# cuulee/reporter

Hardware: AMD Instinct MI355X
Metric: GPS probes matched/sec (whole node) (higher is better)
Workload: dtype f64; 1 GPU; c2; graph=metro, nodes=1048576, directed_edges=3527937, osmlr_segments=1361487, traces_per_gpu=10000, streams=1, device_batches=1, output_segments=1688548

## Files before the change

### reporter_amd/csrc/otr_kernels.h

```cpp
#pragma once
#include <cstddef>
#include <type_traits>

#include "otr_device.h"
#include "otr_mincode.h"
#include "otr_pred.h"
#include "otr_report.h"

#ifndef OTR_CAP1
#define OTR_CAP1 160
#endif
#ifndef OTR_LOAD1
#define OTR_LOAD1 7
#endif
#ifndef OTR_E1CAP
#define OTR_E1CAP 360
#endif
#ifndef OTR_E1LOAD
#define OTR_E1LOAD 14
#endif

namespace otr {

struct BatchDev {
  int32_t n_traces;
  const int64_t* trace_off;
  const double* lat;
  const double* lon;
  const int64_t* time;
  const float* acc;
  const uint8_t* mode;
};

__global__ void k_select_states(BatchDev b, ModeParams mp, int64_t* state_cnt, const int64_t* state_off,
                                int64_t* state_probe, int32_t* state_trace) {
  int t = blockIdx.x * blockDim.x + threadIdx.x;
  if (t >= b.n_traces) return;
  const int64_t lo = b.trace_off[t], hi = b.trace_off[t + 1];
  const MatchParams& P = mp.m[b.mode[t] < OTR_MODES ? b.mode[t] : 0];
  int64_t cnt = 0;
  int64_t base = state_off ? state_off[t] : 0;
  double la_last = 0.0, lo_last = 0.0;
  double la_n = lo < hi ? b.lat[lo] : 0.0, lo_n = lo < hi ? b.lon[lo] : 0.0;
  for (int64_t i = lo; i < hi; ++i) {
    const double la = la_n, lg = lo_n;
    if (i + 1 < hi) {
      la_n = b.lat[i + 1];
      lo_n = b.lon[i + 1];
    }
    const bool st = (i == lo || i == hi - 1) || gc_dist(la_last, lo_last, la, lg) >= P.interpolation_distance;
    if (st) {
      if (state_off) {
        state_probe[base + cnt] = i;
        state_trace[base + cnt] = t;
      }
      ++cnt;
      la_last = la;
      lo_last = lg;
    }
  }
  if (!state_off) state_cnt[t] = cnt;
}

struct CandBuf {
  uint32_t* edge;
  double* p;
  double* sqd;
  int32_t* count;
  double* radius;
};

__device__ inline bool cand_less(double da, uint32_t ea, double db, uint32_t eb) {
  return da < db || (da == db && ea < eb);
}

__device__ inline bool project_edge(const DevGraph& g, uint4 rec, uint4 pts01, uint4 pts23, uint32_t mode_bit,
                                    double plat, double plon, double mpl, double r2, int64_t* sr_out, int64_t* sc_out,
                                    double* d2_out, double* frac_out, unsigned long long* tests) {
  if (!(rec.w & mode_bit)) return false;
  double best = __builtin_huge_val();
  double best_along = 0.0, bqx = 0.0, bqy = 0.0, acc = 0.0;
  const uint32_t k0 = rec.y, k1 = rec.z;
  constexpr uint32_t kPre = 4;
  const int2 pre0 = make_int2((int)pts01.x, (int)pts01.y);
  int2 q1 = make_int2((int)pts01.z, (int)pts01.w);
  int2 q2 = make_int2((int)pts23.x, (int)pts23.y);
  int2 q3 = make_int2((int)pts23.z, (int)pts23.w);
  int2 pa = pre0;
  for (uint32_t k = k0; k + 1 < k1; ++k) {
    const uint32_t i = k + 1 - k0;
    int2 pb;
    if (i < kPre) {
      pb = q1;
      q1 = q2;
      q2 = q3;
    } else {
      pb = g.shape_ll[k + 1];
    }
    const double ax = (e6(pa.y) - plon) * mpl;
    const double ay = (e6(pa.x) - plat) * kMetersPerDeg;
    const double bx = (e6(pb.y) - plon) * mpl;
    const double by = (e6(pb.x) - plat) * kMetersPerDeg;
    const double dx = bx - ax, dy = by - ay;
    const double l2 = dx * dx + dy * dy;
    double t = 0.0;
    if (l2 > 0.0) {
      t = -(ax * dx + ay * dy) / l2;
      if (t < 0.0) t = 0.0;
      if (t > 1.0) t = 1.0;
    }
    const double qx = ax + t * dx, qy = ay + t * dy;
    const double d2 = qx * qx + qy * qy;
    const double sl = sqrt(l2);
    if (d2 < best) {
      best = d2;
      best_along = acc + t * sl;
      bqx = qx;
      bqy = qy;
    }
    acc = acc + sl;
    pa = pb;
  }
  *tests += k1 - k0 - 1;
  if (!(best <= r2)) return false;
  const double slat = plat + bqy / kMetersPerDeg, slon = plon + bqx / mpl;
  *sr_out = (int64_t)floor((slat - g.grid_min_lat) / g.grid_cell_deg);
  *sc_out = (int64_t)floor((slon - g.grid_min_lon) / g.grid_cell_deg);
  *d2_out = best;
  *frac_out = acc > 0.0 ? best_along / acc : 0.0;
  return true;
}

__device__ inline uint32_t wave_sum_u32(uint32_t v) {
  v += (uint32_t)__builtin_amdgcn_update_dpp(0, (int)v, 0x111, 0xf, 0xf, false);
  v += (uint32_t)__builtin_amdgcn_update_dpp(0, (int)v, 0x112, 0xf, 0xf, false);
  v += (uint32_t)__builtin_amdgcn_update_dpp(0, (int)v, 0x114, 0xf, 0xf, false);
  v += (uint32_t)__builtin_amdgcn_update_dpp(0, (int)v, 0x118, 0xf, 0xf, false);
  v += (uint32_t)__builtin_amdgcn_update_dpp(0, (int)v, 0x142, 0xa, 0xf, false);
  v += (uint32_t)__builtin_amdgcn_update_dpp(0, (int)v, 0x143, 0xc, 0xf, false);
  return (uint32_t)__builtin_amdgcn_readlane((int)v, 63);
}

__device__ inline uint32_t wave_min_u32(uint32_t v) {
  const int I = -1;
  auto mn = [](uint32_t a, int b) { return a < (uint32_t)b ? a : (uint32_t)b; };
  v = mn(v, __builtin_amdgcn_update_dpp(I, (int)v, 0x111, 0xf, 0xf, false));
  v = mn(v, __builtin_amdgcn_update_dpp(I, (int)v, 0x112, 0xf, 0xf, false));
  v = mn(v, __builtin_amdgcn_update_dpp(I, (int)v, 0x114, 0xf, 0xf, false));
  v = mn(v, __builtin_amdgcn_update_dpp(I, (int)v, 0x118, 0xf, 0xf, false));
  v = mn(v, __builtin_amdgcn_update_dpp(I, (int)v, 0x142, 0xa, 0xf, false));
  v = mn(v, __builtin_amdgcn_update_dpp(I, (int)v, 0x143, 0xc, 0xf, false));
  return (uint32_t)__builtin_amdgcn_readlane((int)v, 63);
}

__host__ __device__ constexpr bool old_rounds(int g) { return g == 8; }

template <int G>
struct Grp {
  static constexpr int GL = OTR_WAVE / G;
  __device__ static int g() { return G == 1 ? 0 : (int)threadIdx.x / GL; }
  __device__ static int gl() { return G == 1 ? (int)threadIdx.x : (int)threadIdx.x % GL; }
  __device__ static unsigned long long mine(unsigned long long m) {
    return G == 1 ? m : (m >> (GL * g())) & ((1ull << GL) - 1ull);
  }
  __device__ static int prefix(unsigned long long m) {
    if (G == 1) return prefix_count(m);
    return __popcll(mine(m) & ((1ull << gl()) - 1ull));
  }
  __device__ static int count(unsigned long long m) { return __popcll(mine(m)); }
  __device__ static int umax(int v) {
    if (G == 1) return __builtin_amdgcn_readfirstlane(v);
    if (G == 8) {
      int m = __builtin_amdgcn_readlane(v, 0);
#pragma unroll
      for (int q = 1; q < 8; ++q) {
        const int x = __builtin_amdgcn_readlane(v, q * GL);
        m = x > m ? x : m;
      }
      return m;
    }
    const int a = __builtin_amdgcn_readlane(v, 0), b = __builtin_amdgcn_readlane(v, GL);
    if (G == 2) return a > b ? a : b;
    const int c = __builtin_amdgcn_readlane(v, 2 * GL), d = __builtin_amdgcn_readlane(v, 3 * GL);
    const int ab = a > b ? a : b, cd = c > d ? c : d;
    return ab > cd ? ab : cd;
  }
  __device__ static bool all(bool v) {
    if (G == 8) {
      bool r = true;
#pragma unroll
      for (int q = 0; q < 8; ++q) r = r && __builtin_amdgcn_readlane((int)v, q * GL) != 0;
      return r;
    }
    return __ballot(!v) == 0ull;
  }
  __device__ static uint32_t min_u32(uint32_t v) {
    if (G == 1) return wave_min_u32(v);
    if (G == 8) {
#pragma unroll
      for (int o = 1; o < 8; o <<= 1) {
        const uint32_t x = (uint32_t)__shfl_xor((int)v, o, 8);
        v = x < v ? x : v;
      }
      return v;
    }
    const int I = -1;
    auto mn = [](uint32_t a, int b) { return a < (uint32_t)b ? a : (uint32_t)b; };
    v = mn(v, __builtin_amdgcn_update_dpp(I, (int)v, 0x111, 0xf, 0xf, false));
    v = mn(v, __builtin_amdgcn_update_dpp(I, (int)v, 0x112, 0xf, 0xf, false));
    v = mn(v, __builtin_amdgcn_update_dpp(I, (int)v, 0x114, 0xf, 0xf, false));
    v = mn(v, __builtin_amdgcn_update_dpp(I, (int)v, 0x118, 0xf, 0xf, false));
    if (G == 4) {
      const uint32_t a = (uint32_t)__builtin_amdgcn_readlane((int)v, 15);
      const uint32_t b = (uint32_t)__builtin_amdgcn_readlane((int)v, 31);
      const uint32_t c = (uint32_t)__builtin_amdgcn_readlane((int)v, 47);
      const uint32_t d = (uint32_t)__builtin_amdgcn_readlane((int)v, 63);
      const int q = g();
      return q == 0 ? a : (q == 1 ? b : (q == 2 ? c : d));
    }
    v = mn(v, __builtin_amdgcn_update_dpp(I, (int)v, 0x142, 0xa, 0xf, false));
    const uint32_t a = (uint32_t)__builtin_amdgcn_readlane((int)v, 31);
    const uint32_t b = (uint32_t)__builtin_amdgcn_readlane((int)v, 63);
    return g() ? b : a;
  }
};

constexpr int kWin = 16;
#ifndef OTR_CAND2_WAVES
#define OTR_CAND2_WAVES 5
#endif

template <int G>
__global__ __launch_bounds__(64) __attribute__((amdgpu_waves_per_eu(G == 2 ? OTR_CAND2_WAVES : 8, 8))) void k_candidates(
    DevGraph g, BatchDev b, ModeParams mp, int64_t n_states, const int64_t* state_probe, const int32_t* state_trace,
    CandBuf out, unsigned long long* counters) {
  using Gr = Grp<G>;
  constexpr int GL = Gr::GL;
  constexpr int LB = 2 * GL;
  __shared__ double s_d2[G][LB];
  __shared__ double s_p[G][LB];
  __shared__ uint32_t s_e[G][LB];
  __shared__ uint32_t s_bnd[G][kWin][kWin + 1];
  __shared__ uint32_t s_pre[G][kWin + 1];
  const int gi = Gr::g(), lane = Gr::gl();
  const int64_t n_units = (n_states + G - 1) / G;
  const int64_t s = xcd_remap(blockIdx.x, (n_units + 7) / 8) * G + gi;
  if (Gr::umax(s < n_states ? 1 : 0) == 0) return;
  const bool have = s < n_states;
#ifdef OTR_STAMPS_CAND
  const unsigned long long cs0 = __builtin_amdgcn_s_memtime();
  unsigned long long cs1 = cs0, cs2 = cs0;
#endif
  const int64_t probe = have ? state_probe[s] : 0;
  const int mode = have && b.mode[state_trace[s]] < OTR_MODES ? b.mode[state_trace[s]] : 0;
  static_assert(OTR_MODES == 3, "pick() selects among exactly three modes");
  auto pick = [&](auto f) { return mode == 0 ? f(mp.m[0]) : (mode == 1 ? f(mp.m[1]) : f(mp.m[OTR_MODES - 1])); };
  const uint32_t mode_bit = 1u << mode;
  const int kmax = pick([](const MatchParams& q) { return q.kmax; });
  const double plat = b.lat[probe], plon = b.lon[probe];
  const double a = (b.acc && b.acc[probe] >= 0.f) ? (double)b.acc[probe]
                                                  : pick([](const MatchParams& q) { return q.gps_accuracy; });
  const double sr0 = pick([](const MatchParams& q) { return q.search_radius; });
  const double srmax = pick([](const MatchParams& q) { return q.max_search_radius; });
  double radius = sr0 > a ? sr0 : a;
  if (radius > srmax) radius = srmax;
  const double mpl = kMetersPerDeg * cos_deg(plat);
  const double cd = g.grid_cell_deg;
  const double dlat = radius / kMetersPerDeg, dlon = radius / mpl;
  int64_t r0 = (int64_t)floor((plat - dlat - OTR_GRID_PAD_DEG - g.grid_min_lat) / cd);
  int64_t r1 = (int64_t)floor((plat + dlat + OTR_GRID_PAD_DEG - g.grid_min_lat) / cd);
  int64_t c0 = (int64_t)floor((plon - dlon - OTR_GRID_PAD_DEG - g.grid_min_lon) / cd);
  int64_t c1 = (int64_t)floor((plon + dlon + OTR_GRID_PAD_DEG - g.grid_min_lon) / cd);
  if (r0 < 0) r0 = 0;
  if (c0 < 0) c0 = 0;
  if (r1 > (int64_t)g.grid_rows - 1) r1 = (int64_t)g.grid_rows - 1;
  if (c1 > (int64_t)g.grid_cols - 1) c1 = (int64_t)g.grid_cols - 1;
  const double r2 = radius * radius;
  int n = 0;
  unsigned long long tests = 0;
  double* L_d2 = s_d2[gi];
  double* L_p = s_p[gi];
  uint32_t* L_e = s_e[gi];
  auto merge = [&](bool ok, double d2, double frac, uint32_t e) {
    const unsigned long long mask = __ballot(ok);
    if (!mask) return;
    if (ok) {
      const int pos = n + Gr::prefix(mask);
      L_d2[pos] = d2;
      L_p[pos] = frac;
      L_e[pos] = e;
    }
    n += Gr::count(mask);
    __syncthreads();
    if (Gr::umax(n > kmax ? 1 : 0)) {
      double dv[2], pv[2];
      uint32_t ev[2];
      int rk[2];
#pragma unroll
      for (int h = 0; h < 2; ++h) {
        const int idx = lane + h * GL;
        rk[h] = OTR_KMAX * 2;
        if (n > kmax && idx < n) {
          dv[h] = L_d2[idx];
          pv[h] = L_p[idx];
          ev[h] = L_e[idx];
          int rank = 0;
          for (int m = 0; m < n; ++m) rank += cand_less(L_d2[m], L_e[m], dv[h], ev[h]);
          rk[h] = rank;
        }
      }
// ... 1016 lines not shown
    const uint4 r0 = have ? a.rec[3 * task] : make_uint4(0u, 0u, 0u, 0u);
    const uint4 r1 = have ? a.rec[3 * task + 1] : make_uint4(0xFFFFFFFFu, 0u, 0u, 0u);
    const uint4 r2 = have ? a.rec[3 * task + 2] : make_uint4(0u, 0u, 0u, 0u);
    if (lane == 0) {
      trec[Gr::g()][0] = r0;
      trec[Gr::g()][1] = r1;
      trec[Gr::g()][2] = r2;
    }
    const int64_t s = r0.x;
    const unsigned long long mask = ((unsigned long long)r1.w << 32) | r1.z;
    const int64_t sp = r0.y;
    Kb = (int)(r1.y & 0xFFu);
    K.sh = (r1.y >> 11) & 31u;
    const bool general = (r1.y >> 16) & 1u;
    fits = Kb <= Gr::GL && (WIDE || !general) && !((r1.y >> 17) & 1u);
    const bool pre = G >= 2 && !LIST && have && ((r1.y >> 18) & 1u);
    if (pre) {
      start_tier = (int)((r1.y >> 19) & 7u);
      fits = false;
    }
    mode_bit = 1u << ((r1.y >> 8) & 3u);
    bmm = r0.w;
    root = r0.z;
    d0min = r1.x;
    const int32_t bt = (int32_t)r2.y;
    bool needed = false;
    uint4 cq = make_uint4(0u, 0u, 0u, 0u);
    if (have && !pre && lane < Kb) {
      ej = a.cand_edge[s * OTR_KMAX + lane];
      pj = a.cand_p[s * OTR_KMAX + lane];
      cq = a.cprep[s * OTR_KMAX + lane];
      tpart = cq.x;
    }
    const int nsrc = have && !pre ? __popcll(mask) : 0;
    iq = lane < nsrc ? nth_set_bit(mask, lane) : 0;
    if (lane < nsrc) {
      e_q = a.cand_edge[sp * OTR_KMAX + iq];
      p_q = a.cand_p[sp * OTR_KMAX + iq];
      if (bt >= 0) t_q = a.cprep_t[sp * OTR_KMAX + iq].y;
    }
    for (int q = 0; q < nsrc; ++q) {
      uint32_t ei;
      double pi;
      if (q < Gr::GL) {
        ei = (uint32_t)__shfl((int)e_q, q, Gr::GL);
        pi = __shfl(p_q, q, Gr::GL);
      } else {
        const int i = nth_set_bit(mask, q);
        ei = a.cand_edge[sp * OTR_KMAX + i];
        pi = a.cand_p[sp * OTR_KMAX + i];
      }
      if (lane < Kb && !(ej == ei && pj >= pi)) needed = true;
    }
    const uint32_t t0 = (uint32_t)__shfl((int)t_q, 0, Gr::GL);
    bool feasible_root = d0min <= bmm;
    pd = feasible_root ? bmm - d0min : 0u;
    if (bt >= 0) {
      feasible_root = feasible_root && t0 <= (uint32_t)bt;
      pt = t0 <= (uint32_t)bt ? (uint32_t)bt - t0 : 0u;
    }
    forced = have && ((r1.y >> 10) & 1u);
    const unsigned long long need_mask = __ballot(needed);
    search = have && fits && !forced && feasible_root && Gr::mine(need_mask) != 0ull;
    if (needed) {
      tnode = cq.y;
      gapT = cq.z ? cq.z : 1u;
    }
  }
  unsigned long long settled = 0, relaxed = 0, rounds = 0;
  OTR_STAMP(ts_set);
  NDump nd{};
  int dslot = -1;
  constexpr bool kIn = LIST && !WIDE && CAP >= OTR_ND_IN_MIN, kOut = LIST && !WIDE && CAP >= OTR_ND_OUT_MIN;
  constexpr bool kDumps = kIn || kOut;
  if (kIn) {
    const int32_t rs = (a.dump_in != nullptr && search) ? a.task_dump[task] : -1;
    nd.in = rs >= 0 ? a.dump_in + (size_t)rs * a.dump_in_words : nullptr;
  }
  if (kOut) {
    nd.base = a.dump_out;
    nd.ctr = a.dump_ctr;
    nd.words = a.dump_out_words;
    nd.slots = a.dump_out_slots;
#ifdef OTR_FORCE_RETRY
    nd.stop_rounds = (a.force_edge >> 7) & 1 ? 2 + Gr::g() : 0;
#endif
  }
  search_init<CAP, LM, G>(Ls);
  bool ok = search_run<CAP, LM, G, kIn, kOut>(Ls, gr, K, mode_bit, search, root, pd, pt, tnode, tpart, gapT, Kb, &settled,
                                   &relaxed, &rounds, counters ? counters + 16 * kCShards : nullptr, sink,
                                   kDumps ? &nd : nullptr, kDumps ? &dslot : nullptr) &&
            fits;
#ifdef OTR_FORCE_RETRY
  if (G >= 2 && !LIST) ok = false;
#endif
  OTR_STAMP(ts_srch);
  SearchLds<CAP, LM>& L = Ls[Gr::g()];
  int64_t lab = -1;
  if (ok && search && tnode != kEmpty && !forced) {
    const int sl = lds_find(L, tnode);
    if (sl >= 0 && LabelT<LM>::label(L.lab[sl]) != LabelT<LM>::kNone) lab = (int64_t)LabelT<LM>::label(L.lab[sl]);
  }
  asm volatile("" ::: "memory");
  uint32_t ntr = 0;
  if (have && forced && Kb > Gr::GL) {
    const uint4 r1 = trec[Gr::g()][1], r2 = trec[Gr::g()][2];
    const unsigned long long mask = ((unsigned long long)r1.w << 32) | r1.z;
    uint32_t* trow = a.trans + (int64_t)(((uint64_t)r2.w << 32) | r2.z);
    for (int q = 0; q < __popcll(mask); ++q) {
      const int i = nth_set_bit(mask, q);
      for (int j = lane; j < Kb; j += Gr::GL) trow[(int64_t)i * Kb + j] = kNoRoute;
    }
  } else if (have && (ok || forced)) {
    const uint4 r0 = trec[Gr::g()][0], r1 = trec[Gr::g()][1], r2 = trec[Gr::g()][2];
    const int64_t s = r0.x;
    const unsigned long long mask = ((unsigned long long)r1.w << 32) | r1.z;
    if (search) ntr = (uint32_t)Kb * (uint32_t)__popcll(mask);
    const int64_t sp = r0.y;
    const int32_t bt = (int32_t)r2.y;
    uint32_t* trow = a.trans + (int64_t)(((uint64_t)r2.w << 32) | r2.z);
    const int nsrc = __popcll(mask);
    uint32_t w_q = 0;
    uint2 l_q = make_uint2(0u, 0u);
    if (!kKeep) {
      if (!LIST) {
        e_q = t_q = ej = 0u;
        p_q = pj = 0.0;
      }
      iq = lane < nsrc ? nth_set_bit(mask, lane) : 0;
    }
    if (lane < nsrc) {
      if (!kKeep) {
        e_q = a.cand_edge[sp * OTR_KMAX + iq];
        p_q = a.cand_p[sp * OTR_KMAX + iq];
        if (bt >= 0) t_q = a.cprep_t[sp * OTR_KMAX + iq].y;
      }
      w_q = a.cprep[sp * OTR_KMAX + iq].w;
      l_q = a.clen[sp * OTR_KMAX + iq];
    }
    uint32_t tpt = 0;
    if (lane < Kb) {
      if (!kKeep) {
        ej = a.cand_edge[s * OTR_KMAX + lane];
        pj = a.cand_p[s * OTR_KMAX + lane];
      }
      tpt = bt >= 0 ? a.cprep_t[s * OTR_KMAX + lane].x : 0u;
    }
    for (int q = 0; q < nsrc; ++q) {
      int i;
      uint32_t ei, wi, ti, li, lti;
      double pi;
      if (q < Gr::GL) {
        i = __shfl(iq, q, Gr::GL);
        ei = (uint32_t)__shfl((int)e_q, q, Gr::GL);
        pi = __shfl(p_q, q, Gr::GL);
        wi = (uint32_t)__shfl((int)w_q, q, Gr::GL);
        ti = (uint32_t)__shfl((int)t_q, q, Gr::GL);
        li = (uint32_t)__shfl((int)l_q.x, q, Gr::GL);
        lti = (uint32_t)__shfl((int)l_q.y, q, Gr::GL);
      } else {
        i = nth_set_bit(mask, q);
        ei = a.cand_edge[sp * OTR_KMAX + i];
        pi = a.cand_p[sp * OTR_KMAX + i];
        wi = a.cprep[sp * OTR_KMAX + i].w;
        ti = bt >= 0 ? a.cprep_t[sp * OTR_KMAX + i].y : 0u;
        const uint2 l = a.clen[sp * OTR_KMAX + i];
        li = l.x;
        lti = l.y;
      }
      if (lane < Kb) {
        int64_t r = -1, rt = 0;
        if (forced) {
          r = -1;
        } else if (ej == ei && pj >= pi) {
          r = part_mm(pj - pi, li);
          if (bt >= 0) rt = part_mm(pj - pi, lti);
        } else if (lab >= 0) {
          r = (int64_t)wi + K.d((uint64_t)lab) + tpart;
          if (bt >= 0) rt = (int64_t)ti + K.t((uint64_t)lab) + tpt;
        }
        const bool valid = r >= 0 && r <= (int64_t)bmm && (bt < 0 || rt <= (int64_t)bt);
        trow[(int64_t)i * Kb + lane] = valid ? (uint32_t)r : kNoRoute;
      }
    }
  }
  if (have && !ok && !forced && lane == 0) {
    const uint32_t meta = a.rec[3 * task + 1].y;
    const bool general = ((meta >> 16) & 1u) != 0u, turn = ((meta >> 17) & 1u) != 0u;
#ifdef OTR_FORCE_GENERAL
    a.overflow_flag[task] = 3;
#else
    if (!turn) a.overflow_flag[task] = general ? 3 : (start_tier >= 0 ? 16 + start_tier : 1);
#endif
    if (!WIDE && !turn && a.task_dump != nullptr) a.task_dump[task] = dslot;
  }
#ifdef OTR_STAMPS
  if (G == 2 && counters && threadIdx.x == 0) {
    OTR_STAMP(ts_out);
    const int sh = cshard();
    atomicAdd(&counters[20 * kCShards + sh], ts_set - ts_in);
    atomicAdd(&counters[21 * kCShards + sh], ts_out - ts_srch);
  }
#endif
  if (CNT && counters) {
    settled = wave_sum_u32((uint32_t)settled);
    relaxed = wave_sum_u32((uint32_t)relaxed);
    rounds = wave_sum_u32((uint32_t)rounds);
    const int nk = have && search ? L.n_keys : 0;
    unsigned long long kk = 0, ntrw = 0, nsearch = 0, nres = 0, ndmp = 0;
    const int rd = (kDumps && nd.in != nullptr ? 1 : 0) | (dslot >= 0 ? 2 : 0);
    for (int q = 0; q < G; ++q) {
      kk += (unsigned long long)__builtin_amdgcn_readlane(nk, q * Gr::GL);
      ntrw += (unsigned long long)__builtin_amdgcn_readlane(ntr, q * Gr::GL);
      nsearch += (unsigned long long)__builtin_amdgcn_readlane((int)(have && search), q * Gr::GL);
      const int rdq = __builtin_amdgcn_readlane(rd, q * Gr::GL);
      nres += rdq & 1;
      ndmp += rdq >> 1;
    }
    if (threadIdx.x == 0) {
      const int sh = cshard();
      atomicAdd(&counters[3 * kCShards + sh], settled);
      atomicAdd(&counters[4 * kCShards + sh], relaxed);
      atomicAdd(&counters[5 * kCShards + sh], ntrw);
      atomicAdd(&counters[6 * kCShards + sh], nsearch);
      atomicAdd(&counters[13 * kCShards + sh], rounds);
      atomicAdd(&counters[14 * kCShards + sh], kk);
      if (nres) atomicAdd(&counters[11 * kCShards + sh], nres);
      if (ndmp) atomicAdd(&counters[12 * kCShards + sh], ndmp);
    }
  }
}

template <int CAP, int G, bool LIST, bool WIDE = false, bool CNT = true>
__global__ __launch_bounds__(64) __attribute__((amdgpu_waves_per_eu(G == 2 ? OTR_ROUTE2_WAVES : 8, G == 2 ? OTR_ROUTE2_WAVES : 8))) void k_route(DevGraph gr, RouteArgs a, unsigned long long* counters) {
  __shared__ SearchLds<CAP, WIDE ? 2 : 0> Ls[G];
  __shared__ uint4 trec[G][3];
#ifdef OTR_NO_SINK
  uint32_t* sink = nullptr;
#else
  __shared__ uint32_t sink_row[OTR_WAVE];
  uint32_t* sink = WIDE ? nullptr : sink_row;
#endif
  if (!LIST) {
    const int64_t n_units = (a.n_tasks - a.task_base + G - 1) / G;
    const int64_t w = a.unit_base + xcd_remap(blockIdx.x, (int64_t)gridDim.x / 8);
    if (w < n_units) route_unit<CAP, G, LIST, WIDE, CNT>(gr, a, counters, Ls, w, a.n_tasks, sink, trec);
    return;
  }
  const int64_t n_tasks = (int64_t)*a.list_count;
  const int64_t n_units = (n_tasks + G - 1) / G;
  XcdQueue q(a.queue, n_units);
  for (int64_t w = q.next(); w < q.hi; w = q.next()) {
    route_unit<CAP, G, LIST, WIDE, CNT>(gr, a, counters, Ls, w, n_tasks, sink, trec);
    __syncthreads();
  }
}

struct ViterbiArgs {
  int32_t n_traces;
  const int64_t* trace_state_off;
  const int32_t* cand_count;
  const double* cand_sqd;
  const int64_t* prev;
  const int64_t* trans_off;
  const uint32_t* trans;
  const uint32_t* trans_tc;
  uint32_t turn_modes;
  const double* g;
  const uint8_t* mode;
  double inv2s2[OTR_MODES];
  double inv_beta[OTR_MODES];
  int8_t* bp;
  uint8_t* brk;
  int32_t* end_win;
  int32_t* winner;
  int32_t* subpath;
};

__device__ inline double div1000(double x) {
  const double q0 = x * 0.001;
  const double e = __builtin_fma(-q0, 1000.0, x);
  return __builtin_fma(e, 0.001, q0);
}

template <int G>
__device__ inline void argmin_lane(double c, int j, double* oc, int* oj) {
  for (int off = OTR_WAVE / G / 2; off > 0; off >>= 1) {
    const double c2 = __shfl_xor(c, off);
    const int j2 = __shfl_xor(j, off);
    if (c2 < c || (c2 == c && j2 < j)) {
      c = c2;
      j = j2;
    }
  }
  *oc = c;
  *oj = j;
}

template <int G>
struct VitLds {
  static constexpr int N = G == 1 ? 128 : 104;
};

template <bool TURNS, int U = 16>
__device__ __forceinline__ void vit_scan(const uint32_t* tr, const uint32_t* tcr, const double* s_cost, int Kp, int Kw,
                                         int K, int lane, double gcd, double inv_beta, bool turn, double* best_io,
                                         int* bi_io) {
  double best = *best_io;
  int bi = *bi_io;
  for (int i0 = 0; i0 < Kw; i0 += U) {
    uint32_t tv[U], tc[U];
#pragma unroll
    for (int u = 0; u < U; ++u) {
      const int i = i0 + u < Kp ? i0 + u : Kp - 1;
      tv[u] = tr[(int64_t)i * K + lane];
    }
#pragma unroll
    for (int u = 0; u < U; ++u) {
      const int i = i0 + u < Kp ? i0 + u : Kp - 1;
      tc[u] = (TURNS && turn) ? tcr[(int64_t)i * K + lane] : 0u;
    }
#pragma unroll
    for (int u = 0; u < U; ++u) {
      if (i0 + u >= Kp || tv[u] == kNoRoute) continue;
      const double dg = fabs(div1000((double)tv[u]) - gcd);
      const double ti = (TURNS ? div1000((double)tc[u]) + dg : dg) * inv_beta;
      const double ci = s_cost[i0 + u < Kp ? i0 + u : Kp - 1];
      if (ci == __builtin_huge_val()) continue;
      const double c = ci + ti;
      if (c < best) {
        best = c;
        bi = i0 + u;
      }
    }
  }
  *best_io = best;
  *bi_io = bi;
}

template <bool TURNS, int U = 8>
__device__ __forceinline__ void vit_scan_half(const uint32_t* tr, const uint32_t* tcr, const double* s_cost, int Kp,
                                              int K, int j, int h, double gcd, double inv_beta, bool turn,
                                              double* best_io, int* bi_io) {
  double best = *best_io;
  int bi = *bi_io;
  for (int i0 = h; i0 < Kp; i0 += 2 * U) {
    uint32_t tv[U], tc[U];
#pragma unroll
    for (int u = 0; u < U; ++u) {
      const int i = i0 + 2 * u < Kp ? i0 + 2 * u : Kp - 1;
      tv[u] = tr[(int64_t)i * K + j];
    }
#pragma unroll
    for (int u = 0; u < U; ++u) {
      const int i = i0 + 2 * u < Kp ? i0 + 2 * u : Kp - 1;
      tc[u] = (TURNS && turn) ? tcr[(int64_t)i * K + j] : 0u;
    }
#pragma unroll
    for (int u = 0; u < U; ++u) {
      if (i0 + 2 * u >= Kp || tv[u] == kNoRoute) continue;
      const double dg = fabs(div1000((double)tv[u]) - gcd);
      const double ti = (TURNS ? div1000((double)tc[u]) + dg : dg) * inv_beta;
      const double ci = s_cost[i0 + 2 * u];
      if (ci == __builtin_huge_val()) continue;
      const double c = ci + ti;
      if (c < best) {
        best = c;
        bi = i0 + 2 * u;
      }
    }
  }
  *best_io = best;
  *bi_io = bi;
}
__device__ __forceinline__ void vit_pair(double* best, int* bi) {
  const double ob = __shfl_xor(*best, 32);
  const int obi = __shfl_xor(*bi, 32);
  if (obi >= 0 && (*bi < 0 || ob < *best || (ob == *best && obi < *bi))) {
    *best = ob;
    *bi = obi;
  }
}

template <int G, bool SPLIT = false>
__global__ __launch_bounds__(64) void k_viterbi(ViterbiArgs a, unsigned long long* counters) {
  static_assert(!SPLIT || G == 1, "the split scan uses the second half of a one-trace wave");
  constexpr int GL = OTR_WAVE / G;
  constexpr int NL = VitLds<G>::N;
  __shared__ double s_cost[G][OTR_KMAX / G];
  __shared__ int8_t s_bp[G][NL][32];
  __shared__ int8_t s_brk[G][NL];
  __shared__ int8_t s_win[G][NL];
  const int gi = G == 1 ? 0 : (int)threadIdx.x / GL;
  const int lane = G == 1 ? (int)threadIdx.x : (int)threadIdx.x % GL;
  double* const cst = s_cost[gi];
  for (int64_t tw = blockIdx.x; tw * G < a.n_traces; tw += gridDim.x) {
    const int64_t t = tw * G + gi;
    const bool have = t < a.n_traces;
    const int md = have && a.mode[t] < OTR_MODES ? a.mode[t] : 0;
    const double inv2s2 = a.inv2s2[md], inv_beta = a.inv_beta[md];
    const bool turns = (a.turn_modes >> md) & 1u;
    const bool wturns = G == 1 ? turns : __ballot(turns) != 0ull;
    const int64_t so = have ? a.trace_state_off[t] : 0, eo = have ? a.trace_state_off[t + 1] : 0;
    int64_t len = eo - so;
    if (G == 2) {
      const int64_t l0 = __builtin_amdgcn_readlane((int)len, 0), l1 = __builtin_amdgcn_readlane((int)len, 32);
      len = l0 > l1 ? l0 : l1;
    }
    int64_t prev_s = -1;
    int Kp = 0;
    bool lds_ok = eo - so <= NL;
    for (int64_t k = 0; k < len; ++k) {
      const int Kw = G == 1 ? Kp : max(__builtin_amdgcn_readlane(Kp, 0), __builtin_amdgcn_readlane(Kp, 32));
      const int64_t s = so + k;
      const bool in = s < eo;
      const int K = in ? a.cand_count[s] : 0;
      if (in && lds_ok && lane == 0) s_brk[gi][k] = -1;
      const bool act = in && K > 0;
      if (act) lds_ok = lds_ok && K <= 32;
      double emis = 0.0;
      if (act && lane < K) emis = a.cand_sqd[s * OTR_KMAX + lane] * inv2s2;
      double cost = __builtin_huge_val();
      int bi = -1;
      bool brk = prev_s < 0;
      if (act && !brk) {
        double best = __builtin_huge_val();
        const bool split = SPLIT && K <= 32;
        if (split) {
          const uint32_t* tr = a.trans + a.trans_off[s];
          const uint32_t* tcr = a.trans_tc + a.trans_off[s];
          const double gcd = a.g[s];
          const int j = lane & 31;
          if (j < K) {
            if (wturns) vit_scan_half<true>(tr, tcr, cst, Kp, K, j, lane >> 5, gcd, inv_beta, turns, &best, &bi);
            else vit_scan_half<false>(tr, tcr, cst, Kp, K, j, lane >> 5, gcd, inv_beta, false, &best, &bi);
          }
          vit_pair(&best, &bi);
          if (lane >= 32) {
            best = __builtin_huge_val();
            bi = -1;
          }
        } else if (lane < K) {
          const uint32_t* tr = a.trans + a.trans_off[s];
          const uint32_t* tcr = a.trans_tc + a.trans_off[s];
          const double gcd = a.g[s];
          if (wturns) vit_scan<true, G == 1 ? 16 : 8>(tr, tcr, cst, Kp, Kw, K, lane, gcd, inv_beta, turns, &best, &bi);
          else vit_scan<false, G == 1 ? 16 : 8>(tr, tcr, cst, Kp, Kw, K, lane, gcd, inv_beta, false, &best, &bi);
        }
        const unsigned long long am = __ballot(lane < K && bi >= 0);
        const bool any = (G == 1 ? am : (am >> (GL * gi)) & ((1ull << GL) - 1ull)) != 0ull;
        if (!any) {
          brk = true;
          bi = -1;
        } else {
          cost = bi >= 0 ? best + emis : __builtin_huge_val();
        }
      }
      double mc;
      int mj;
      argmin_lane<G>(lane < Kp ? cst[lane] : __builtin_huge_val(), lane < Kp ? lane : OTR_KMAX, &mc, &mj);
      if (act && brk) {
        if (prev_s >= 0) {
          if (lane == 0) a.end_win[prev_s] = mj;
          if (lds_ok && lane == 0) s_win[gi][prev_s - so] = (int8_t)mj;
        }
        cost = emis;
        bi = -1;
      }
      if (act) {
        if (lane < K) a.bp[s * OTR_KMAX + lane] = (int8_t)bi;
        if (lane == 0) a.brk[s] = brk ? 1 : 0;
        if (lds_ok) {
          if (lane < K) s_bp[gi][k][lane] = (int8_t)bi;
          if (lane == 0) s_brk[gi][k] = brk ? 1 : 0;
        }
      }
      __syncthreads();
      if (act && lane < K) cst[lane] = cost;
      __syncthreads();
      if (act) {
        prev_s = s;
        Kp = K;
      }
    }
    {
      double mc;
      int mj;
      argmin_lane<G>(lane < Kp ? cst[lane] : __builtin_huge_val(), lane < Kp ? lane : OTR_KMAX, &mc, &mj);
      if (prev_s >= 0) {
        if (lane == 0) a.end_win[prev_s] = mj;
        if (lds_ok && lane == 0) s_win[gi][prev_s - so] = (int8_t)mj;
      }
    }
    __syncthreads();
    if (have && lds_ok && lane == 0) {
      int cur = -1;
      bool next_brk = true;
      for (int64_t s = eo - 1; s >= so; --s) {
        const int k = (int)(s - so);
        const int b = s_brk[gi][k];
        if (b < 0) {
          a.winner[s] = -1;
          continue;
        }
        if (next_brk) cur = s_win[gi][k];
        a.winner[s] = cur;
        if (!b) cur = s_bp[gi][k][cur];
        next_brk = b != 0;
      }
      int sp = -1;
      for (int64_t s = so; s < eo; ++s) {
        const int b = s_brk[gi][s - so];
        sp += b > 0 ? 1 : 0;
        a.subpath[s] = b < 0 ? -1 : sp;
      }
    } else if (have && lane == 0) {
      int cur = -1;
      bool next_brk = true;
      for (int64_t s = eo - 1; s >= so; --s) {
        if (a.cand_count[s] <= 0) {
          a.winner[s] = -1;
          a.subpath[s] = -1;
          continue;
        }
        if (next_brk) cur = a.end_win[s];
        a.winner[s] = cur;
        const bool b = a.brk[s] != 0;
        if (!b) cur = a.bp[s * OTR_KMAX + cur];
        next_brk = b;
      }
      int sp = -1;
      for (int64_t s = so; s < eo; ++s) {
        if (a.cand_count[s] <= 0) continue;
        if (a.brk[s]) ++sp;
        a.subpath[s] = sp;
      }
    }
    __syncthreads();
  }
  (void)counters;
}

struct PathArgs {
  const int64_t* steps;
  int64_t n_steps;
  const int64_t* prev;
  const double* bound;
  const uint8_t* brk;
  const int32_t* winner;
  const uint32_t* cand_edge;
  const double* cand_p;
  const int32_t* state_trace;
  const uint8_t* mode;
  const uint4* cprep;
  const uint2* cprep_t;
  const int32_t* bt;
  uint32_t turn_modes;
  const unsigned long long* n_steps_dev;
  int64_t* path_off;
  int32_t* path_len;
  uint32_t* path;
  unsigned long long* cursor;
  int64_t capacity;
  int32_t* overflow_flag;
  int32_t* cap_flag;
  const int32_t* cand_count;
  const int64_t* trans_off;
  const uint32_t* trans;
  int force_edge;
  unsigned long long* queue;
  bool from_back;
};

struct PathClass {
  const int32_t* winner;
  const int64_t* trans_off;
  const uint32_t* trans;
  const double* bound;
  const int32_t* state_trace;
  const uint8_t* mode;
  uint32_t turn_modes;
  float est4;
  float small_keys;
};

template <int CAP, int G>
__global__ __launch_bounds__(64) __attribute__((amdgpu_waves_per_eu(G >= 2 ? 6 : 8, 8))) void k_paths(DevGraph gr, PathArgs a, const int64_t* step_list, const unsigned long long* list_count) {
  using Gr = Grp<G>;
  __shared__ SearchLds<CAP, true> Ls[G];
  const int gl = Gr::gl();
  const int64_t n_list = (int64_t)(step_list ? *list_count : *a.n_steps_dev);
  const int64_t n_units = (n_list + G - 1) / G;
  XcdQueue q(a.queue, step_list ? n_units : 0);
  const int64_t wend = step_list ? q.hi : n_units;
  for (int64_t w = step_list ? q.next() : xcd_remap(blockIdx.x, gridDim.x / 8); w < wend;
       w = step_list ? q.next() : wend) {
  const int64_t iw = w * G + Gr::g();
  const bool have = iw < n_list;
  const int64_t k = have ? (step_list ? step_list[iw] : (a.from_back ? a.n_steps - n_list + iw : iw)) : 0;
  const int64_t s = have ? a.steps[k] : 0;
  const int64_t sp = have ? a.prev[s] : 0;
  bool active = false;
  uint32_t S = 0, T = kEmpty, bmm = 0, tpart = 0, gapT = 1, d0 = 0, mode_bit = 1, pd = 0, pt = 0xFFFFFFFFu;
  int mode = 0;
  Pack K;
  K.sh = 0;
  if (have) {
    const int wi = a.winner[sp], wj = a.winner[s];
    const uint32_t ei = a.cand_edge[sp * OTR_KMAX + wi], ej = a.cand_edge[s * OTR_KMAX + wj];
    const double pi = a.cand_p[sp * OTR_KMAX + wi], pj = a.cand_p[s * OTR_KMAX + wj];
    mode = a.mode[a.state_trace[s]] < OTR_MODES ? a.mode[a.state_trace[s]] : 0;
    bmm = (uint32_t)bound_mm_of(a.bound[s]);
    {
      const uint32_t r = a.trans[a.trans_off[s] + (int64_t)wi * a.cand_count[s] + wj];
      if (r < bmm) bmm = r;
    }
    const int32_t bt = a.bt[s];
    K.sh = pack_shift(bt);
    if (ej == ei && pj >= pi) {
      if (gl == 0) a.path_len[s] = -1;
    } else if (((a.turn_modes >> mode) & 1u)
#ifdef OTR_FORCE_GENERAL
               && false
#endif
    ) {
      if (gl == 0) a.overflow_flag[k] = 5;
    } else if (!pack_fits(bmm, K.sh)
#ifdef OTR_FORCE_GENERAL
               || true
#endif
    ) {
      if (gl == 0) a.overflow_flag[k] = 3;
    } else {
      active = true;
      mode_bit = 1u << mode;
      const uint4 cs = a.cprep[sp * OTR_KMAX + wi], ct = a.cprep[s * OTR_KMAX + wj];
      d0 = cs.w;
      pd = bmm >= d0 ? bmm - d0 : 0u;
      if (bt >= 0) {
        const uint32_t t0 = a.cprep_t[sp * OTR_KMAX + wi].y;
        pt = t0 <= (uint32_t)bt ? (uint32_t)bt - t0 : 0u;
      }
      S = gr.edge_dst[ei];
      T = ct.y;
      gapT = ct.z ? ct.z : 1u;
      tpart = ct.x;
    }
  }
  search_init<CAP, true, G>(Ls);
  const bool ok = search_run<CAP, true, G>(Ls, gr, K, mode_bit, active, S, pd, pt, gl == 0 ? T : kEmpty, tpart, gapT,
                                           1, nullptr, nullptr, nullptr);
  SearchLds<CAP, true>& L = Ls[Gr::g()];
  if (active && !ok) {
    if (gl == 0) a.overflow_flag[k] = 1;
    active = false;
  }
  static_assert(sizeof(L.pend) + sizeof(L.work) >= 4 * CAP, "predecessor nodes reuse pend + work");
  using PL = SearchLds<CAP, true>;
  static_assert(offsetof(PL, work) == offsetof(PL, pend) + sizeof(L.pend), "pend and work are contiguous");
  uint32_t* pn = reinterpret_cast<uint32_t*>(L.pend);
  constexpr int kPer = (CAP + Gr::GL - 1) / Gr::GL;
  if (active) {
    for (int r0 = 0; r0 < kPer; r0 += 8) {
      uint32_t u[8];
#pragma unroll
      for (int r = 0; r < 8; ++r) {
        const int q = gl + (r0 + r) * Gr::GL;
        u[r] = kEmpty;
        if (q < CAP && L.key[q] != kEmpty) {
          const uint32_t e = (uint32_t)(L.lab[q] & 0xFFFFFFFFull);
          if (e != kEmpty) u[r] = gr.edge_src[e];
        }
      }
#pragma unroll
      for (int r = 0; r < 8; ++r)
        if (gl + (r0 + r) * Gr::GL < CAP) pn[gl + (r0 + r) * Gr::GL] = u[r];
    }
  }
  __syncthreads();
  int n = 0;
  if (active && gl == 0) {
    uint32_t v = T;
    while (v != S) {
      const int sv = lds_find(L, v);
      const uint32_t e = sv >= 0 ? (uint32_t)(L.lab[sv] & 0xFFFFFFFFull) : kEmpty;
      if (e == kEmpty || n >= CAP) {
        n = -1;
        break;
      }
      ++n;
      v = pn[sv];
    }
  }
  n = __shfl(n, Gr::g() * Gr::GL);
  if (active && n < 0) {
    if (gl == 0) a.overflow_flag[k] = 1;
    active = false;
  }
  const int shard = (int)((blockIdx.x * G + Gr::g()) & (kShards - 1));
  const int64_t region = a.capacity / kShards;
  int64_t off = 0;
  if (active && gl == 0) off = (int64_t)atomicAdd(&a.cursor[shard], (unsigned long long)n);
  off = __shfl(off, Gr::g() * Gr::GL);
  if (active && off + n > region) {
    if (gl == 0) *a.cap_flag = 1;
    active = false;
  }
  if (active && gl == 0) {
    off += (int64_t)shard * region;
    uint32_t v = T;
    for (int q = n - 1; q >= 0; --q) {
      const int sv = lds_find(L, v);
      a.path[off + q] = (uint32_t)(L.lab[sv] & 0xFFFFFFFFull);
      v = pn[sv];
    }
    a.path_off[s] = off;
    a.path_len[s] = n;
  }
  __syncthreads();
  }
}

struct SegArgs {
  BatchDev b;
  const int64_t* trace_state_off;
  const int64_t* state_probe;
  const int32_t* cand_count;
  const uint32_t* cand_edge;
  const double* cand_p;
  const int64_t* prev;
  const uint8_t* brk;
  const int32_t* winner;
  const int64_t* path_off;
  const int32_t* path_len;
  const uint32_t* path;
  int64_t* pos;
  int64_t* ent;
  int64_t* act;
  int32_t* suba;
  int32_t* subb;
  uint32_t* por_e;  int64_t* por_s0;  int64_t* por_s1;  int32_t* por_sa;  int32_t* gstart;
  const int64_t* cap_off;
  int64_t n_traces_pad;
  uint32_t* route;  int64_t* route_n;
  unsigned long long* seg_id;  double* seg_start;  double* seg_end;  int32_t* seg_length;
  int32_t* seg_queue;  uint8_t* seg_internal;  int32_t* seg_bshape;  int32_t* seg_eshape;
  uint32_t* seg_index;  int64_t* seg_n;
  int64_t* seg_way_n;  uint32_t* seg_way;  int64_t* way_n;
  unsigned long long* rep_id;  unsigned long long* rep_next;  double* rep_t0;  double* rep_t1;
  int32_t* rep_length;  int32_t* rep_queue;  uint32_t* rep_seg;  int64_t* rep_n;
  int32_t* shape_used;  int32_t* stats;  double* stats_len;
  double threshold;
  uint32_t report_levels, transition_levels;
  double queue_kph[OTR_MODES];
};

template <class T>
__device__ inline T wave_excl_sum(T v, T* total) {
  const int lane = threadIdx.x;
  T x = v;
  for (int off = 1; off < OTR_WAVE; off <<= 1) {
    const T u = __shfl_up(x, off);
    if (lane >= off) x += u;
  }
  *total = __shfl(x, OTR_WAVE - 1);
  return x - v;
}

__device__ inline bool group_continues(const DevGraph& g, uint32_t ep, uint32_t e) {
  const uint32_t key = g.edge_seg[ep];
  if (key != OTR_NO_SEGMENT)
    return g.edge_seg[e] == key && !(g.edge_attr[ep] & OTR_ATTR_SEG_END) && !(g.edge_attr[e] & OTR_ATTR_SEG_BEGIN);
  return g.edge_seg[e] == OTR_NO_SEGMENT &&
         ((g.edge_attr[e] & OTR_ATTR_INTERNAL) != 0) == ((g.edge_attr[ep] & OTR_ATTR_INTERNAL) != 0);
}

__global__ __launch_bounds__(64) void k_segments(DevGraph g, SegArgs a, unsigned long long* counters) {
  const int lane = threadIdx.x;
  const int64_t t = xcd_remap(blockIdx.x, (a.b.n_traces + 7) / 8);
  if (t >= a.b.n_traces) return;
  const int64_t so = a.trace_state_off[t], eo = a.trace_state_off[t + 1];
  const int64_t lo_probe = a.b.trace_off[t], n_probe = a.b.trace_off[t + 1] - lo_probe;
  const int64_t co = a.cap_off[t];
  const double qkph = a.queue_kph[a.b.mode[t] < OTR_MODES ? a.b.mode[t] : 0];
  int64_t* act = a.act + so;
  int64_t* pos = a.pos + so;
  int64_t* ent = a.ent + so;
  int32_t* suba = a.suba + so;
  int32_t* subb = a.subb + so;
  int na = 0;
  for (int64_t base = so; base < eo; base += OTR_WAVE) {
    const int64_t s = base + lane;
    const bool on = s < eo && a.cand_count[s] > 0;
    const unsigned long long m = __ballot(on);
    if (on) act[na + prefix_count(m)] = s;
    na += __popcll(m);
  }
  __syncthreads();
  int64_t c_pos = 0, c_ent = 0, n_por = 0, n_route = 0;
  int c_sa = 0;
  bool emitted_any = false;
  for (int kb = 0; kb < na; kb += OTR_WAVE) {
    const int k = kb + lane;
    const bool valid = k < na;
    int64_t s = 0;
    bool brk_k = false, last_k = false, same = false, change = false;
    uint32_t ek = 0, ep = 0;
    double pk = 0, pp = 0;
    int pl = 0;
    int64_t inc = 0;
    if (valid) {
      s = act[k];
      brk_k = a.brk[s] != 0;
      last_k = (k == na - 1) || a.brk[act[k + 1]] != 0;
      ek = a.cand_edge[s * OTR_KMAX + a.winner[s]];
      pk = a.cand_p[s * OTR_KMAX + a.winner[s]];
      if (!brk_k) {
        const int64_t sp = act[k - 1];
        ep = a.cand_edge[sp * OTR_KMAX + a.winner[sp]];
        pp = a.cand_p[sp * OTR_KMAX + a.winner[sp]];
        same = ek == ep && pk >= pp;
        change = !same;
      }
      if (same) inc = part_mm(pk - pp, g.len_mm[ep]);
      if (change) {
        pl = a.path_len[s];
        inc = part_mm(1.0 - pp, g.len_mm[ep]);
        for (int z = 0; z < pl; ++z) inc += (int64_t)g.len_mm[a.path[a.path_off[s] + z]];
        inc += part_mm(pk, g.len_mm[ek]);
      }
    }
    int64_t v = inc;
    bool f = brk_k;
    for (int off = 1; off < OTR_WAVE; off <<= 1) {
      const int64_t vu = __shfl_up(v, off);
      const bool fu = __shfl_up((int)f, off) != 0;
      if (lane >= off) {
        if (!f) v += vu;
// ... 535 lines not shown
```

Before: 35.90 million probes/s.

## Software-pipeline Viterbi step loads and stage backtrace results in LDS

New measurement: 35.91 million probes/s (median of 2 runs). Within noise of the previous version (+0.0%).

```diff
diff --git a/reporter_amd/csrc/otr_kernels.h b/reporter_amd/csrc/otr_kernels.h
--- a/reporter_amd/csrc/otr_kernels.h
+++ b/reporter_amd/csrc/otr_kernels.h
@@ -6,6 +6,7 @@
 #include "otr_mincode.h"
 #include "otr_pred.h"
 #include "otr_report.h"
+#include "otr_vit_plan.h"
 
 #ifndef OTR_CAP1
 #define OTR_CAP1 160
@@ -1628,77 +1629,65 @@
   static constexpr int N = G == 1 ? 128 : 104;
 };
 
-template <bool TURNS, int U = 16>
-__device__ __forceinline__ void vit_scan(const uint32_t* tr, const uint32_t* tcr, const double* s_cost, int Kp, int Kw,
-                                         int K, int lane, double gcd, double inv_beta, bool turn, double* best_io,
-                                         int* bi_io) {
+__device__ __forceinline__ uint32_t vit_idx(int row, int K, int col) {
+  return __umul24((uint32_t)row, (uint32_t)K) + (uint32_t)col;
+}
+
+template <bool TURNS, int U>
+__device__ __forceinline__ void vit_eval(const uint32_t (&tv)[U], const uint32_t (&tc)[U], const double* s_cost,
+                                         int base, VitLane l, int Kp, int Kw, double gcd, double inv_beta,
+                                         double* best_io, int* bi_io) {
   double best = *best_io;
   int bi = *bi_io;
-  for (int i0 = 0; i0 < Kw; i0 += U) {
+#pragma unroll
+  for (int u = 0; u < U; ++u) {
+    if (base + l.stride * u >= Kw) break;
+    const int i = base + l.first + l.stride * u;
+    if (i >= Kp || tv[u] == kNoRoute) continue;
+    const double dg = fabs(div1000((double)tv[u]) - gcd);
+    const double ti = (TURNS ? div1000((double)tc[u]) + dg : dg) * inv_beta;
+    const double ci = s_cost[i];
+    if (ci == __builtin_huge_val()) continue;
+    const double c = ci + ti;
+    if (c < best) {
+      best = c;
+      bi = i;
+    }
+  }
+  *best_io = best;
+  *bi_io = bi;
+}
+
+template <int UP>
+struct VitRows {
+  uint32_t tv[UP];
+  double sqd, g;
+};
+
+template <bool TURNS, int U, int UP>
+__device__ __forceinline__ void vit_scan_rest(const uint32_t* tr, const uint32_t* tcr, const double* s_cost, int Kp,
+                                              int Kw, int K, VitLane l, double gcd, double inv_beta, bool turn,
+                                              double* best_io, int* bi_io) {
+  for (int base = l.stride * UP; base < Kw; base += l.stride * U) {
     uint32_t tv[U], tc[U];
 #pragma unroll
     for (int u = 0; u < U; ++u) {
-      const int i = i0 + u < Kp ? i0 + u : Kp - 1;
-      tv[u] = tr[(int64_t)i * K + lane];
+      const int i = base + l.first + l.stride * u;
+      tv[u] = tr[vit_idx(i < Kp ? i : Kp - 1, K, l.col)];
     }
 #pragma unroll
-    for (int u = 0; u < U; ++u) {
-      const int i = i0 + u < Kp ? i0 + u : Kp - 1;
-      tc[u] = (TURNS && turn) ? tcr[(int64_t)i * K + lane] : 0u;
-    }
+    for (int u = 0; u < U; ++u) tc[u] = 0u;
+    if (TURNS && turn) {
 #pragma unroll
-    for (int u = 0; u < U; ++u) {
-      if (i0 + u >= Kp || tv[u] == kNoRoute) continue;
-      const double dg = fabs(div1000((double)tv[u]) - gcd);
-      const double ti = (TURNS ? div1000((double)tc[u]) + dg : dg) * inv_beta;
-      const double ci = s_cost[i0 + u < Kp ? i0 + u : Kp - 1];
-      if (ci == __builtin_huge_val()) continue;
-      const double c = ci + ti;
-      if (c < best) {
-        best = c;
-        bi = i0 + u;
-      }
-    }
-  }
-  *best_io = best;
-  *bi_io = bi;
-}
-
-template <bool TURNS, int U = 8>
-__device__ __forceinline__ void vit_scan_half(const uint32_t* tr, const uint32_t* tcr, const double* s_cost, int Kp,
-                                              int K, int j, int h, double gcd, double inv_beta, bool turn,
-                                              double* best_io, int* bi_io) {
-  double best = *best_io;
-  int bi = *bi_io;
-  for (int i0 = h; i0 < Kp; i0 += 2 * U) {
-    uint32_t tv[U], tc[U];
-#pragma unroll
-    for (int u = 0; u < U; ++u) {
-      const int i = i0 + 2 * u < Kp ? i0 + 2 * u : Kp - 1;
-      tv[u] = tr[(int64_t)i * K + j];
-    }
-#pragma unroll
-    for (int u = 0; u < U; ++u) {
-      const int i = i0 + 2 * u < Kp ? i0 + 2 * u : Kp - 1;
-      tc[u] = (TURNS && turn) ? tcr[(int64_t)i * K + j] : 0u;
-    }
-#pragma unroll
-    for (int u = 0; u < U; ++u) {
-      if (i0 + 2 * u >= Kp || tv[u] == kNoRoute) continue;
-      const double dg = fabs(div1000((double)tv[u]) - gcd);
-      const double ti = (TURNS ? div1000((double)tc[u]) + dg : dg) * inv_beta;
-      const double ci = s_cost[i0 + 2 * u];
-      if (ci == __builtin_huge_val()) continue;
-      const double c = ci + ti;
-      if (c < best) {
-        best = c;
-        bi = i0 + 2 * u;
-      }
-    }
-  }
-  *best_io = best;
-  *bi_io = bi;
-}
+      for (int u = 0; u < U; ++u) {
+        const int i = base + l.first + l.stride * u;
+        tc[u] = tcr[vit_idx(i < Kp ? i : Kp - 1, K, l.col)];
+      }
+    }
+    vit_eval<TURNS, U>(tv, tc, s_cost, base, l, Kp, Kw, gcd, inv_beta, best_io, bi_io);
+  }
+}
+
 __device__ __forceinline__ void vit_pair(double* best, int* bi) {
   const double ob = __shfl_xor(*best, 32);
   const int obi = __shfl_xor(*bi, 32);
@@ -1709,69 +1698,112 @@
 }
 
 template <int G, bool SPLIT = false>
-__global__ __launch_bounds__(64) void k_viterbi(ViterbiArgs a, unsigned long long* counters) {
+__global__ __launch_bounds__(64, SPLIT ? 4 : 5) void k_viterbi(ViterbiArgs a, unsigned long long* counters) {
   static_assert(!SPLIT || G == 1, "the split scan uses the second half of a one-trace wave");
+  static_assert(kVitMetaAhead == 2 && kVitRowsAhead == 1, "the loop below is written for these depths");
   constexpr int GL = OTR_WAVE / G;
   constexpr int NL = VitLds<G>::N;
+  constexpr int U = G == 1 ? 16 : 8;
+  constexpr int UP = kVitPreRows;
   __shared__ double s_cost[G][OTR_KMAX / G];
   __shared__ int8_t s_bp[G][NL][32];
   __shared__ int8_t s_brk[G][NL];
   __shared__ int8_t s_win[G][NL];
-  const int gi = G == 1 ? 0 : (int)threadIdx.x / GL;
-  const int lane = G == 1 ? (int)threadIdx.x : (int)threadIdx.x % GL;
-  double* const cst = s_cost[gi];
+  static_assert(NL <= 128, "sub-path ordinals (0 .. NL - 1) of an LDS-cached trace fit an int8");
   for (int64_t tw = blockIdx.x; tw * G < a.n_traces; tw += gridDim.x) {
+    int tid = (int)__lane_id();
+    asm volatile("" : "+v"(tid));
+    const int gi = G == 1 ? 0 : tid / GL;
+    const int lane = G == 1 ? tid : tid % GL;
+    double* const cst = s_cost[gi];
     const int64_t t = tw * G + gi;
     const bool have = t < a.n_traces;
     const int md = have && a.mode[t] < OTR_MODES ? a.mode[t] : 0;
     const double inv2s2 = a.inv2s2[md], inv_beta = a.inv_beta[md];
     const bool turns = (a.turn_modes >> md) & 1u;
     const bool wturns = G == 1 ? turns : __ballot(turns) != 0ull;
-    const int64_t so = have ? a.trace_state_off[t] : 0, eo = have ? a.trace_state_off[t + 1] : 0;
-    int64_t len = eo - so;
+    const int64_t so = have ? a.trace_state_off[t] : 0;
+    const int n = have ? (int)(a.trace_state_off[t + 1] - so) : 0;
+    int len = n;
     if (G == 2) {
-      const int64_t l0 = __builtin_amdgcn_readlane((int)len, 0), l1 = __builtin_amdgcn_readlane((int)len, 32);
+      const int l0 = __builtin_amdgcn_readlane(len, 0), l1 = __builtin_amdgcn_readlane(len, 32);
       len = l0 > l1 ? l0 : l1;
     }
-    int64_t prev_s = -1;
-    int Kp = 0;
-    bool lds_ok = eo - so <= NL;
-    for (int64_t k = 0; k < len; ++k) {
+    auto load_count = [&](int k) { return vit_state_in(k, n) ? a.cand_count[so + k] : 0; };
+    auto load_rows = [&](int k, int K, VitChain before, int64_t toff) {
+      VitRows<UP> r;
+      r.sqd = 0.0;
+      r.g = 0.0;
+#pragma unroll
+      for (int u = 0; u < UP; ++u) r.tv[u] = kNoRoute;
+      if (vit_active(K) && lane < K) r.sqd = a.cand_sqd[(so + k) * OTR_KMAX + lane];
+      if (vit_scans(before, K)) {
+        r.g = a.g[so + k];
+        const VitLane l = vit_lane(vit_split(SPLIT, K), lane, K);
+        if (l.on) {
+          const uint32_t* tr = a.trans + toff;
+#pragma unroll
+          for (int u = 0; u < UP; ++u) r.tv[u] = tr[vit_idx(vit_row(l, u, before.Kp), K, l.col)];
+        }
+      }
+      return r;
+    };
+    VitChain ch = vit_chain_start();
+    int K0 = load_count(0), K1 = load_count(1);
+    int64_t toff = n > 0 ? a.trans_off[so] : 0;
+    VitRows<UP> r = load_rows(0, K0, ch, toff);
+    bool lds_ok = n <= NL;
+    for (int k = 0; k < len; ++k) {
+      const int64_t prev_s = ch.prev < 0 ? -1 : so + ch.prev;
+      const int Kp = ch.Kp;
       const int Kw = G == 1 ? Kp : max(__builtin_amdgcn_readlane(Kp, 0), __builtin_amdgcn_readlane(Kp, 32));
       const int64_t s = so + k;
-      const bool in = s < eo;
-      const int K = in ? a.cand_count[s] : 0;
+      const bool in = vit_state_in(k, n);
+      const int K = K0;
+      const bool act = vit_active(K);
+      const VitChain ch1 = vit_chain_next(ch, k, K);
+      const int64_t toff1 = toff + vit_block_words(ch, K);
       if (in && lds_ok && lane == 0) s_brk[gi][k] = -1;
-      const bool act = in && K > 0;
       if (act) lds_ok = lds_ok && K <= 32;
       double emis = 0.0;
-      if (act && lane < K) emis = a.cand_sqd[s * OTR_KMAX + lane] * inv2s2;
+      if (act && lane < K) emis = r.sqd * inv2s2;
       double cost = __builtin_huge_val();
       int bi = -1;
       bool brk = prev_s < 0;
+      const bool split = vit_split(SPLIT, K);
+      const VitLane l = vit_lane(split, lane, K);
+      const double gcd = r.g;
+      const uint32_t* tr = a.trans + toff;
+      const uint32_t* tcr = a.trans_tc + toff;
+      double best = __builtin_huge_val();
+      if (act && !brk && l.on) {
+        uint32_t tc[UP];
+#pragma unroll
+        for (int u = 0; u < UP; ++u) tc[u] = 0u;
+        if (wturns && turns) {
+#pragma unroll
+          for (int u = 0; u < UP; ++u) tc[u] = tcr[vit_idx(vit_row(l, u, Kp), K, l.col)];
+        }
+        const int Ke = SPLIT && split ? Kp : Kw;
+        if (wturns) vit_eval<true, UP>(r.tv, tc, cst, 0, l, Kp, Ke, gcd, inv_beta, &best, &bi);
+        else vit_eval<false, UP>(r.tv, tc, cst, 0, l, Kp, Ke, gcd, inv_beta, &best, &bi);
+      }
+      const int K2 = load_count(k + kVitMetaAhead);
+      r = load_rows(k + kVitRowsAhead, K1, ch1, toff1);
       if (act && !brk) {
-        double best = __builtin_huge_val();
-        const bool split = SPLIT && K <= 32;
-        if (split) {
-          const uint32_t* tr = a.trans + a.trans_off[s];
-          const uint32_t* tcr = a.trans_tc + a.trans_off[s];
-          const double gcd = a.g[s];
-          const int j = lane & 31;
-          if (j < K) {
-            if (wturns) vit_scan_half<true>(tr, tcr, cst, Kp, K, j, lane >> 5, gcd, inv_beta, turns, &best, &bi);
-            else vit_scan_half<false>(tr, tcr, cst, Kp, K, j, lane >> 5, gcd, inv_beta, false, &best, &bi);
+        if (SPLIT && split) {
+          if (l.on) {
+            if (wturns) vit_scan_rest<true, 8, UP>(tr, tcr, cst, Kp, Kp, K, l, gcd, inv_beta, turns, &best, &bi);
+            else vit_scan_rest<false, 8, UP>(tr, tcr, cst, Kp, Kp, K, l, gcd, inv_beta, false, &best, &bi);
           }
           vit_pair(&best, &bi);
           if (lane >= 32) {
             best = __builtin_huge_val();
             bi = -1;
           }
-        } else if (lane < K) {
-          const uint32_t* tr = a.trans + a.trans_off[s];
-          const uint32_t* tcr = a.trans_tc + a.trans_off[s];
-          const double gcd = a.g[s];
-          if (wturns) vit_scan<true, G == 1 ? 16 : 8>(tr, tcr, cst, Kp, Kw, K, lane, gcd, inv_beta, turns, &best, &bi);
-          else vit_scan<false, G == 1 ? 16 : 8>(tr, tcr, cst, Kp, Kw, K, lane, gcd, inv_beta, false, &best, &bi);
+        } else if (l.on) {
+          if (wturns) vit_scan_rest<true, U / 2, UP>(tr, tcr, cst, Kp, Kw, K, l, gcd, inv_beta, turns, &best, &bi);
+          else vit_scan_rest<false, U, UP>(tr, tcr, cst, Kp, Kw, K, l, gcd, inv_beta, false, &best, &bi);
         }
         const unsigned long long am = __ballot(lane < K && bi >= 0);
         const bool any = (G == 1 ? am : (am >> (GL * gi)) & ((1ull << GL) - 1ull)) != 0ull;
@@ -1804,12 +1836,14 @@
       __syncthreads();
       if (act && lane < K) cst[lane] = cost;
       __syncthreads();
-      if (act) {
-        prev_s = s;
-        Kp = K;
-      }
+      ch = ch1;
+      toff = toff1;
+      K0 = K1;
+      K1 = K2;
     }
     {
+      const int64_t prev_s = ch.prev < 0 ? -1 : so + ch.prev;
+      const int Kp = ch.Kp;
       double mc;
       int mj;
       argmin_lane<G>(lane < Kp ? cst[lane] : __builtin_huge_val(), lane < Kp ? lane : OTR_KMAX, &mc, &mj);
@@ -1822,25 +1856,25 @@
     if (have && lds_ok && lane == 0) {
       int cur = -1;
       bool next_brk = true;
-      for (int64_t s = eo - 1; s >= so; --s) {
-        const int k = (int)(s - so);
+      for (int k = n - 1; k >= 0; --k) {
         const int b = s_brk[gi][k];
         if (b < 0) {
-          a.winner[s] = -1;
+          s_win[gi][k] = -1;
           continue;
         }
         if (next_brk) cur = s_win[gi][k];
-        a.winner[s] = cur;
+        s_win[gi][k] = (int8_t)cur;
         if (!b) cur = s_bp[gi][k][cur];
         next_brk = b != 0;
       }
       int sp = -1;
-      for (int64_t s = so; s < eo; ++s) {
-        const int b = s_brk[gi][s - so];
+      for (int k = 0; k < n; ++k) {
+        const int b = s_brk[gi][k];
         sp += b > 0 ? 1 : 0;
-        a.subpath[s] = b < 0 ? -1 : sp;
+        s_brk[gi][k] = (int8_t)(b < 0 ? -1 : sp);
       }
     } else if (have && lane == 0) {
+      const int64_t eo = so + n;
       int cur = -1;
       bool next_brk = true;
       for (int64_t s = eo - 1; s >= so; --s) {
@@ -1860,6 +1894,13 @@
         if (a.cand_count[s] <= 0) continue;
         if (a.brk[s]) ++sp;
         a.subpath[s] = sp;
+      }
+    }
+    __syncthreads();
+    if (have && lds_ok) {
+      for (int k = lane; k < n; k += GL) {
+        a.winner[so + k] = s_win[gi][k];
+        a.subpath[so + k] = s_brk[gi][k];
       }
     }
     __syncthreads();
diff --git a/reporter_amd/csrc/otr_vit_plan.h b/reporter_amd/csrc/otr_vit_plan.h
--- /dev/null
+++ b/reporter_amd/csrc/otr_vit_plan.h
@@ -0,0 +1,43 @@
+#pragma once
+#include <hip/hip_runtime.h>
+
+#include <cstdint>
+
+namespace otr {
+
+constexpr int kVitMetaAhead = 2;
+constexpr int kVitRowsAhead = 1;
+constexpr int kVitPreRows = 6;
+
+__host__ __device__ inline bool vit_state_in(int k, int n) { return k >= 0 && k < n; }
+
+struct VitChain {
+  int Kp;
+  int prev;
+};
+__host__ __device__ inline VitChain vit_chain_start() { return VitChain{0, -1}; }
+__host__ __device__ inline bool vit_active(int K) { return K > 0; }
+__host__ __device__ inline VitChain vit_chain_next(VitChain c, int k, int K) {
+  return vit_active(K) ? VitChain{K, k} : c;
+}
+__host__ __device__ inline bool vit_scans(VitChain before, int K) { return vit_active(K) && before.prev >= 0; }
+__host__ __device__ inline int64_t vit_block_words(VitChain before, int K) {
+  return vit_scans(before, K) ? (int64_t)before.Kp * K : 0;
+}
+__host__ __device__ inline bool vit_split(bool split_kernel, int K) { return split_kernel && K <= 32; }
+
+struct VitLane {
+  bool on;
+  int col, first, stride;
+};
+__host__ __device__ inline VitLane vit_lane(bool split, int lane, int K) {
+  const int col = split ? lane & 31 : lane;
+  return VitLane{col < K, col, split ? lane >> 5 : 0, split ? 2 : 1};
+}
+__host__ __device__ inline int vit_row(VitLane l, int u, int Kp) {
+  const int r = l.first + l.stride * u;
+  return r < Kp ? r : Kp - 1;
+}
+__host__ __device__ inline int vit_word(int row, int K, int col) { return row * K + col; }
+
+}
```
